# mwhoffman/pybo

Hardware: AMD Instinct MI355X
Metric: BO-step wall-clock (GP fit + 1e6-candidate acq sweep) at N obs; steps/sec (higher is better)
Workload: dtype f64

## Files before the change

pybo_amd/csrc/api.hip:

```cpp
#include <math.h>
#include <stdio.h>
#include <stdlib.h>
#include <string.h>

#include <algorithm>
#include <cmath>
#include <functional>
#include <new>

#include "gpx_internal.h"
#include "gpx_diag.h"
#include "acq_core.h"
#include "mes_math.h"
#include "kg_math.h"

using namespace gpx;

static thread_local std::string g_create_err;

#define HIPCHK(h, call)                                                                     \
    do {                                                                                    \
        hipError_t e_ = (call);                                                             \
        if (e_ != hipSuccess) {                                                             \
            char buf_[512];                                                                 \
// ... 99 lines not shown
    void (*set)(gpx_handle* h, int64_t v);
    bool (*ok)(int64_t v) = nullptr;
    const char* bad_ok = nullptr;
};
template <int gpx_handle::*F>
static void store(gpx_handle* h, int64_t v) { h->*F = (int)v; }
static bool mult128(int64_t v) { return v % 128 == 0; }
static const int64_t BIG = INT64_MAX;
static const char* const TG = "chol_tg*: out of range";
static const char* const TRTRI = "trtri_ahead*: out of range";
static const char* const XBG = "x_bg*: out of range";
static const Option kOptions[] = {
    {"chunk", SHIP, 128, BIG, "chunk must be a positive multiple of 128", [](gpx_handle* h, int64_t v) { h->chunk = v; }, mult128},
    {"super_m", SHIP, 1, 16, "super_m must be 1, 2, 4, 8 or 16", store<&gpx_handle::super_m>, [](int64_t v) { return (v & (v - 1)) == 0; }},
    {"tile_order", SHIP, -1, 31, "tile_order: -1 (by size) or bits 0-1 tile map (0..3), bits 2-4 k-loop schedule (1 .. 7)",
     store<&gpx_handle::tile_order>, [](int64_t v) { return v == -1 || v >= 4; }},
    {"sweep_cache", SHIP, -1, 1, "sweep_cache must be 1, 0 or -1",
     [](gpx_handle* h, int64_t v) { h->cache_on = (v == 1); if (v < 0) { h->cache_valid = false; h->npend = 0; } }},
    {"prune", SHIP, -1, 1, "prune must be -1 (by size and gate), 0 (never) or 1 (wherever legal)", store<&gpx_handle::prune>},
    {"prune_keep", DIAG, 0, 1, "prune_keep must be 0 or 1", store<&gpx_handle::prune_keep>},
    {"prune_bound", DIAG, -1, 2, "prune_bound must be -1 (by guard), 0 (generic kernel), 1 (matrix-pipe kernel) or 2 (fp32 matrix-pipe kernel)", store<&gpx_handle::prune_bound>},
    {"bound_fact", DIAG, 0, 1, "bound_fact must be 0 (the fp32 bound kernel never takes its factorised form) or 1 (by its guard)", store<&gpx_handle::bound_fact>},
    {"prune_rows", DIAG, -1, 1000000, "prune_rows must be -1 (by size), 0 (no second bound) or a number of block rows", store<&gpx_handle::prune_rows>},
    {"short_map", DIAG, -1, 1, "short_map must be -1 (by size), 0 (never) or 1 (wherever tile map 3 is in use)", store<&gpx_handle::short_map>},
    {"chol_w", SHIP, 0, 8, "chol_w must be 0 (by size) or in [2, 8]", store<&gpx_handle::chol_w>, [](int64_t v) { return v != 1; }},
    {"chol_tg", SHIP, -1, 1000000000, TG, store<&gpx_handle::chol_tg>, [](int64_t v) { return v == 0 || v == 1; }, "chol_tg must be 0 or 1"},
    {"chol_tg_chunks", DIAG, -1, 1000000000, TG, store<&gpx_handle::tg_chunks>},
    {"chol_tg_grid", DIAG, -1, 1000000000, TG, store<&gpx_handle::tg_grid>},
    {"chol_tg_trace", DIAG, -1, 1000000000, TG, store<&gpx_handle::tg_trace>},
    {"chol_tg_isolate", DIAG, -1, 1000000000, TG, store<&gpx_handle::tg_isolate>},
    {"chol_tg_nap", DIAG, -1, 1000000000, TG, [](gpx_handle* h, int64_t v) { h->tg_nap = (int)std::max<int64_t>(0, std::min<int64_t>(127, v)); }},
    {"chol_tg_tmo_ms", SHIP, -1, 1000000000, TG, store<&gpx_handle::tg_tmo_ms>},
    {"chol_tg_min", SHIP, -1, 1000000000, TG, [](gpx_handle* h, int64_t v) { h->tg_min = (int)std::max<int64_t>(1, v); }},
    {"chol_tg_max", SHIP, -1, 1000000000, TG, [](gpx_handle* h, int64_t v) { h->tg_max = (int)std::max<int64_t>(1, v); }},
    {"chol_tg_db", SHIP, -1, 1000000000, TG, [](gpx_handle* h, int64_t v) { h->tg_db = (v < 0) ? -1 : (v != 0 ? 1 : 0); }},
    {"chol_tg_db_max", SHIP, -1, 1000000000, TG, [](gpx_handle* h, int64_t v) { h->tg_db_max = (int)std::max<int64_t>(0, v); }},
    {"chol_tg_fuse", SHIP, -1, 1000000000, TG, [](gpx_handle* h, int64_t v) { h->tg_fuse = (v != 0) ? 1 : 0; }},
    {"trtri_ahead", SHIP, 0, 1000000, TRTRI, [](gpx_handle* h, int64_t v) { h->trtri_ahead = (v != 0) ? 1 : 0; }},
    {"trtri_ahead_min", SHIP, 0, 1000000, TRTRI, [](gpx_handle* h, int64_t v) { h->trtri_ahead_min = (int)std::max<int64_t>(4, v); }},
    {"chol_fuse", SHIP, 0, 1, "chol_fuse must be 0 or 1", store<&gpx_handle::chol_fuse>},
    {"chol_graph", SHIP, 0, 1, "chol_graph must be 0 or 1", store<&gpx_handle::chol_graph>},
    {"chol_merge", SHIP, 0, 100000, "chol_merge: 0 (off) or a minimum number of block rows", store<&gpx_handle::chol_merge>},
    {"chol_rl", SHIP, 0, 1, "chol_rl must be 0 or 1", store<&gpx_handle::chol_rl>},
    {"x_skip", DIAG, 0, 7, "x_skip: bits 0..2", store<&gpx_handle::x_skip>},
    {"x_bg", DIAG, 0, 10000000, XBG, store<&gpx_handle::x_bg>},
    {"x_bg_lds", DIAG, 0, 10000000, XBG, store<&gpx_handle::x_bg_lds>},
// ... 839 lines not shown
    const int64_t nx = Xc ? M * h->d : 0;
    int rc;
    if ((rc = ensure(h, h->dXc, h->cap_xc, staged_ws(WsCarver(nullptr), nx, M).bytes / 8))) return rc;
    const StagedWs st = staged_ws(WsCarver(h->dXc), nx, M);
    if (Xc) {
        Span sp(h, T_COPY);
        HIPCHK(h, hipMemcpyAsync(st.X, Xc, (size_t)nx * 8, hipMemcpyHostToDevice, h->stream));
    }
    if (sync_upload) HIPCHK(h, hipStreamSynchronize(h->stream));
    if ((rc = core(st.X, acq_all ? st.acq : nullptr, mu ? st.mu : nullptr, s2 ? st.s2 : nullptr))) return rc;
    {
        Span sp(h, T_COPY);
        if (acq_all) HIPCHK(h, hipMemcpyAsync(acq_all, st.acq, (size_t)M * 8, hipMemcpyDeviceToHost, h->stream));
        if (mu) HIPCHK(h, hipMemcpyAsync(mu, st.mu, (size_t)M * 8, hipMemcpyDeviceToHost, h->stream));
        if (s2) HIPCHK(h, hipMemcpyAsync(s2, st.s2, (size_t)M * 8, hipMemcpyDeviceToHost, h->stream));
    }
    HIPCHK(h, hipStreamSynchronize(h->stream));
    return GPX_OK;
}

static const int64_t PRUNE_MIN_M = 32768, PRUNE_MIN_NP = 1024, PRUNE_MAX_SHARE_DIV = 4;
static const double PRUNE_GATE_S2 = 1.0 / 64.0;
static const int PRUNE_ROWS_MIN_NP = 32, PRUNE_ROWS_DIV = 4;

struct PruneGeom { int64_t G, Gg, cap; };
static PruneGeom prune_geom(int nP, int64_t k, int64_t M) {
    const int64_t gen_tiles = std::max<int64_t>(1, 512 / ((nP + 1) / 2));
    const int64_t G0 = (int64_t)TBH * std::min<int64_t>(32, gen_tiles);
    const int64_t G = std::max<int64_t>(G0, (k + TBH - 1) / TBH * TBH);
    return {G, (int64_t)TBH * gen_tiles, std::max<int64_t>(G, M / PRUNE_MAX_SHARE_DIV)};
}

static int prune_ws(gpx_handle* h, int64_t M, int64_t cap, int64_t Gg, int64_t extra, PruneWs& w, bool rows = false) {
    const int64_t need = prune_ws_layout(WsCarver(nullptr), M, cap, h->d, h->Np, Gg, extra, rows).bytes;
    if (!h->dprune || need > h->cap_prune) h->ens_rec = gpx_handle::EnsPruneRecord();
    if (int rc = ensure(h, h->dprune, h->cap_prune, need)) return rc;
    w = prune_ws_layout(WsCarver(h->dprune), M, cap, h->d, h->Np, Gg, extra, rows);
    return GPX_OK;
}

static const int64_t BOUND_F32_MIN_M = 131072;
static void bound_dots(gpx_handle* h, const double* dXc, int64_t M, const PruneWs& w, bool bound_mfma, double* out) {
    hipStream_t s = h->stream;
    launch_prune_alpha(s, h->dU, h->Np, h->da, h->rho, h->bias, w.alpha2, w.sabs, w.sc);
    if (bound_mfma)
        launch_bound_mfma(s, h->dXs, h->N, h->Np, (int)h->d, w.alpha2, h->rho, dXc, M, h->dinvell, h->prune_bound, M >= BOUND_F32_MIN_M, h->bound_fact != 0,
                          w.bws, w.sc, out);
    launch_sweep_rank1_v(s, h->dXs, h->N, (int)h->d, w.alpha2, h->Np, w.sc + 2, dXc, M, h->dinvell, h->kernel_id, h->rho,
                         nullptr, out, bound_mfma ? w.sc + 9 : nullptr);
}

static int64_t sweep_chunk(const gpx_handle* h, int64_t M) {
    const int64_t chunk_opt = h->chunk > 0 ? h->chunk : (h->Np <= 4096 ? 131072 : 65536);
    return std::min<int64_t>(chunk_opt, (M + TBH - 1) / TBH * TBH);
}

struct SelectList { const double* X; int64_t* idx; int64_t n; };
struct SelectOps {
    std::function<int(const double* X, int64_t mb, int64_t me, double* out, double* mu, double* s2)> exact;
    std::function<int(int64_t Gg, double* value, bool* go)> gate;
    std::function<int(double* ub, int64_t done)> bound;
    std::function<int()> after_seeds;
    std::function<int(SelectList& list)> refine;
};

template <typename Rec>
static int select_topk_pruned(gpx_handle* L, bool legal, bool selection_only, int acq_id, int n, int nP, int64_t Np_min, const double* dXc,
                              int64_t M, int64_t k, int64_t ws_extra, bool ws_rows, PruneWs& w, PruneHint& hint, Rec& rec, double* out,
                              const SelectOps& ops, int64_t* done) {
    const PruneGeom geom = prune_geom(nP, k, M);
    const int64_t G = geom.G, Gg = geom.Gg, cap = geom.cap;
    const Rec fresh = rec;
    auto start_rec = [&]() {
        rec = fresh;
        rec.path = 0, rec.M = M, rec.k = k, rec.G = G, rec.Gg = Gg, rec.cap = cap, rec.gate = NAN;
    };
    start_rec();
    *done = 0;
    legal = legal && selection_only && acq_id == GPX_ACQ_EI && k > 0 && L->prune != 0 && M >= 3 * G;
    bool pruning = legal && (L->prune == 1 || (M >= PRUNE_MIN_M && Np_min >= PRUNE_MIN_NP && M >= Gg + 2 * G));
    if (!pruning) return GPX_OK;
    hipStream_t s = L->stream;
    int rc;
    const int64_t kk = std::min<int64_t>(k, TOPK_PASS);
    if ((rc = ensure(L, L->dblkv, L->cap_blk, topk_blocks(M) * kk))) return rc;
    if ((rc = ensure(L, L->dblki, L->cap_blki, topk_blocks(M) * kk))) return rc;
    if ((rc = ensure(L, L->dtopv, L->cap_top, (int64_t)TOPK_MAX * 2))) return rc;
    L->dtopi = reinterpret_cast<int64_t*>(L->dtopv + TOPK_MAX);
    if ((rc = prune_ws(L, M, cap, Gg, ws_extra, w, ws_rows))) return rc;
    start_rec();
    PruneHint key;
    key.kernel_id = L->kernel_id, key.n = n, key.d = L->d, key.nP = nP, key.Np_min = Np_min, key.M = M, key.k = k;
    const bool automatic = L->prune < 0;
// ... 122 lines not shown
        h->npend = 0;
        if ((rc = ensure(h, h->dcZ, h->cap_cz, M * h->d))) return rc;
        if ((rc = ensure(h, h->dcq, h->cap_cq, 2 * M))) return rc;
        h->dcp = h->dcq + h->cap_cq / 2;
        cq = h->dcq;
        cp = h->dcp;
        if (dXc != h->dcZ)
            HIPCHK(h, hipMemcpyAsync(h->dcZ, dXc, (size_t)M * h->d * 8, hipMemcpyDeviceToDevice, s));
    }

    const int sweep_order = h->tile_order >= 0 ? h->tile_order : (Np / NB < 32 ? 7 : 19);

    auto run_chunks = [&](const double* X, int64_t mb, int64_t me, double* out, double* mu, double* s2) -> int {
        for (int64_t m0 = mb; m0 < me; m0 += chunk) {
            const int64_t valid = std::min(chunk, me - m0);
            const int64_t cols = (valid + TBH - 1) / TBH * TBH;
            {
                Span sp(h, T_XGRAM);
                launch_cross_gram(s, h->dXs, Np, h->N, (int)h->d, X, m0, me, cols, h->dinvell, h->kernel_id,
                                  h->rho, h->dKs, Np);
            }
            {
                Span sp(h, T_TRMM);
                launch_sweep_trmm(s, h->dU, Np, nP, h->dKs, chunk, cols, h->da, h->dQp, h->dPp, chunk, sweep_order, h->super_m, h->dclk, h->short_map);
            }
            h->tacc[T_NLAUNCH] += 1.0;
            h->tacc[T_FLOP] += (double)h->N * (double)h->N * (double)valid;
            {
                Span sp(h, T_ACQ);
                if (kg) {
                    launch_kg_cross(s, kb.B, Np, h->dKs, Np, cols, h->dkgw, chunk);
                    launch_acq_kg(s, h->dQp, h->dPp, chunk, nP, m0, valid, h->rho, h->bias, h->sn2, h->kernel_id, (int)h->d, X, h->dinvell,
                                  kb.As, kb.m, kb.al, h->dkgw, chunk, out, mu, s2, cq, cp);
                } else if (mes) launch_acq_mes(s, h->dQp, h->dPp, chunk, nP, m0, valid, h->rho, h->bias, ys, out, mu, s2, cq, cp);
                else launch_acq(s, h->dQp, h->dPp, chunk, nP, m0, valid, h->rho, h->bias, acq_id, p0, out, mu, s2, cq, cp);
            }
        }
        return GPX_OK;
    };

    gpx_handle::PruneRecord& rec = h->prune_rec;
    PruneWs w;
    KeepWs kw = {};
    SelectOps ops;
    ops.exact = run_chunks;
    ops.gate = [&](int64_t Gg, double* value, bool* go) -> int {
        run_chunks(dXc, 0, Gg, d_acq, nullptr, w.gs2);
// ... 8 lines not shown
    ops.bound = [&](double* ub, int64_t done) -> int {
        const bool bound_mfma = h->prune_bound != 0 && bound_mfma_ks(h->kernel_id, (int)h->d) > 0;
        {
            Span sp(h, T_BOUND);
            bound_dots(h, dXc, M, w, bound_mfma, w.dots);
            if (h->prune_keep) {
                if ((rc = ensure(h, h->dkeep, h->cap_keep, keep_ws(WsCarver(nullptr), M, rec.G).bytes))) return rc;
                kw = keep_ws(WsCarver(h->dkeep), M, rec.G);
                HIPCHK(h, hipMemcpyAsync(kw.dots, w.dots, (size_t)M * 8, hipMemcpyDeviceToDevice, s));
            }
            launch_prune_ub(s, w.dots, ub, M, done, w.sc, h->rho, h->bias, p0);
        }
        rec.bound_kernel = bound_mfma ? -1 : 0, rec.st = w.st, rec.kept = h->prune_keep != 0;
        if (rec.kept) HIPCHK(h, hipMemcpyAsync(kw.ub, ub, (size_t)M * 8, hipMemcpyDeviceToDevice, s));
        return GPX_OK;
    };
    ops.after_seeds = [&]() -> int {
        if (rec.kept) HIPCHK(h, hipMemcpyAsync(kw.seed, w.idx, (size_t)rec.G * 8, hipMemcpyDeviceToDevice, s));
        return GPX_OK;
    };
    ops.refine = [&](SelectList& list) -> int { return second_bound(h, w, chunk, sweep_order, p0, list); };
    int64_t done = 0;
    const bool legal = !h->cache_on && h->rho >= gpx::S2_FLOOR && h->rho < INFINITY;
    if ((rc = select_topk_pruned(h, legal, selection_only, acq_id, 1, nP, Np, dXc, M, k, 0, true, w, h->prune_hint, rec, d_acq, ops, &done)))
        return rc;
    if ((rc = plain_rest(ops, dXc, done, chunk, M, d_acq, d_mu, d_s2))) return rc;
    if (h->cache_on) {
        h->cache_valid = true;
        h->cache_M = M;
    }
    if (k > 0 && (rc = topk_core(h, d_acq, M, k, top_val, top_idx))) return rc;
    HIPCHK(h, hipGetLastError());
    return GPX_OK;
}

extern "C" int gpx_sweep_dev(gpx_handle* h, int acq_id, const double* params, int nparams, const double* dXc,
                             int64_t M, int64_t k, double* top_val, int64_t* top_idx, double* d_acq_all,
                             double* d_mu, double* d_s2) {
    return guarded(h, [&]() -> int {
        if (!h) return GPX_EARG;
        return sweep_core(h, acq_id, params, nparams, dXc, M, k, top_val, top_idx, d_acq_all, d_mu, d_s2);
    });
}

extern "C" int gpx_sweep(gpx_handle* h, int acq_id, const double* params, int nparams, const double* Xc,
                         int64_t M, int64_t k, double* top_val, int64_t* top_idx, double* acq_all, double* mu,
                         double* s2) {
// ... 588 lines not shown
            PruneWs wm = w;
            if (h != L) {
                h->prune_rec = gpx_handle::PruneRecord();
                if ((rc = prune_ws(h, 0, 0, 0, 0, wm))) return member_fail(L, h, m, rc);
            }
            {
                Span sp(h, T_BOUND);
                const bool bound_mfma = h->prune_bound != 0 && bound_mfma_ks(h->kernel_id, (int)h->d) > 0;
                bound_dots(h, dXc, M, wm, bound_mfma, t1);
                launch_prune_ub_fold(h->stream, t1, ub, M, wm.sc, h->rho, h->bias, params[0], m == 0, delta + m,
                                     bound_mfma ? 1 : 0, delta + n + m);
            }
            HIPCHK(L, hipStreamSynchronize(h->stream));
        }
        {
            Span sp(L, T_BOUND);
            launch_prune_ub_mean(s, ub, M, done, (double)n);
        }
        rec.delta = delta;
        return GPX_OK;
    };
    ops.after_seeds = [&]() -> int { HIPCHK(L, hipStreamSynchronize(s)); return GPX_OK; };
    int64_t done = 0;
    if ((rc = select_topk_pruned(L, members_ok, !d_out && !d_mu && !d_s2, acq_id, n, nPmax, Np_min, dXc, M, k, 3 * n, false, w, L->ens_hint, rec,
                                 out, ops, &done)))
        return rc;
    if ((rc = plain_rest(ops, dXc, done, sweep_chunk(L, M), M, out, d_mu, d_s2))) return rc;
    if (k > 0) {
        if ((rc = topk_core(L, out, M, k, top_val, top_idx))) return rc;
    } else {
        HIPCHK(L, hipStreamSynchronize(L->stream));
    }
    HIPCHK(L, hipGetLastError());
    return GPX_OK;
}

static int ensemble_check(gpx_handle* const* members, int n) {
    if (!members || n < 1 || !members[0]) return GPX_EARG;
    for (int m = 1; m < n; ++m)
        if (!members[m]) {
            members[0]->err = "ensemble_sweep: NULL member handle";
            return GPX_EARG;
        }
    return GPX_OK;
}

extern "C" int gpx_ensemble_predict(gpx_handle* const* members, int n_members, const double* Xc, int64_t M,
// ... 254 lines not shown
```

pybo_amd/csrc/gemm_core.h:

```cpp
#pragma once
#include <hip/hip_runtime.h>
#include <stdint.h>
#include <type_traits>

namespace gpx {

typedef double d4 __attribute__((ext_vector_type(4)));
typedef double d2 __attribute__((ext_vector_type(2)));

constexpr int TB = 128;
constexpr int BK = 16;
constexpr int LDT = TB + 16;
constexpr int GEMM_THREADS = 256;
constexpr int GEMM_LDS_F64 = 2 * 2 * BK * LDT;
constexpr int GEMM_LDS_BYTES = GEMM_LDS_F64 * 8;

__device__ __forceinline__ void acc_zero(d4 (&acc)[4][4]) {
#pragma unroll
    for (int i = 0; i < 4; ++i)
#pragma unroll
        for (int j = 0; j < 4; ++j) acc[i][j] = (d4){0.0, 0.0, 0.0, 0.0};
}

struct LaunchClock {
    const unsigned long long c0, r0;
    __device__ __forceinline__ LaunchClock() : c0(__builtin_readcyclecounter()), r0(wall_clock64()) {}
    __device__ __forceinline__ void add(unsigned long long* clk) const {
        if (clk && threadIdx.x == 0) {
            atomicAdd(clk, (unsigned long long)__builtin_readcyclecounter() - c0);
            atomicAdd(clk + 1, (unsigned long long)wall_clock64() - r0);
        }
    }
};

template <bool PRIO, bool ILV = false>
__device__ __forceinline__ void gemm_tile_128_b(d4 (&acc)[4][4], const double* __restrict__ A, int64_t lda,
                                                const double* __restrict__ B, int64_t ldb, int k_lo,
                                                int k_hi, double* smem) {
    const int t = threadIdx.x;
    const int lane = t & 63;
    const int w = t >> 6;
    const int wm = w >> 1, wn = w & 1;
    double* As = smem;
    double* Bs = smem + 2 * BK * LDT;
// ... 289 lines not shown
            if (W2) {
                ra[kk] = __builtin_bit_cast(d2, __builtin_amdgcn_raw_buffer_load_b128(rA, voA, kk * soA, AUX));
                rb[kk] = __builtin_bit_cast(d2, __builtin_amdgcn_raw_buffer_load_b128(rB, voB, kk * soB, AUX));
                __builtin_amdgcn_sched_group_barrier(0x020, 2, 0);
            }
        }
        if (W2) {
            Abase += (int64_t)BK32 * lda * 8;
            Bbase += (int64_t)BK32 * ldb * 8;
        }
        __syncthreads();
    };
    int kt = 0;
    for (; kt + 2 < nk; ++kt) step(kt, std::true_type{}, std::true_type{});
    if (kt + 1 < nk) { step(kt, std::true_type{}, std::false_type{}); ++kt; }
    step(kt, std::false_type{}, std::false_type{});
    if (PRIO) __builtin_amdgcn_s_setprio(PRIO - 1);
}

typedef __attribute__((address_space(3))) void* gemm_lds_ptr;
template <int BKL>
constexpr int gemm_l_lds_f64() { return 2 * BKL * LDT; }

template <int BKL, int PRIO = 1, int NSET = 2, bool ILV = false, bool TRI = false, bool NEGA = false, int AUX = 0, bool REV = false>
__device__ __forceinline__ void gemm_tile_128_l(d4 (&acc)[4][4], const double* __restrict__ A, int64_t lda,
                                                const double* __restrict__ B, int64_t ldb, int k_lo, int k_hi,
                                                double* smem) {
    static_assert(!TRI || ILV, "TRI needs the interleaved row blocks");
    static_assert(!REV || BKL == 32, "REV is the order of the 32-row steps: gemm_rev32 for other step sizes");
    constexpr int G = BKL / 4;
    const int lane = threadIdx.x & 63;
    const int w = __builtin_amdgcn_readfirstlane(threadIdx.x >> 6);
    const int wm = w >> 1, wn = w & 1;
    double* As = smem;
    double* Bs = smem + BKL * LDT;
    const int nk = (k_hi - k_lo) / BKL;
    if (nk <= 0) return;
    const char* Abase = reinterpret_cast<const char*>(A + (int64_t)(REV ? k_hi - BKL : k_lo) * lda);
    const char* Bbase = reinterpret_cast<const char*>(B + (int64_t)(REV ? k_hi - BKL : k_lo) * ldb);
    const int64_t stepA = (REV ? -1 : 1) * (int64_t)BKL * lda * 8, stepB = (REV ? -1 : 1) * (int64_t)BKL * ldb * 8;
    const int voA = (int)(((int64_t)w * lda + 2 * lane) * 8), voB = (int)(((int64_t)w * ldb + 2 * lane) * 8);
    const int soA = (int)(4 * lda * 8), soB = (int)(4 * ldb * 8);
    auto issue = [&]() {
        __amdgpu_buffer_rsrc_t rA = __builtin_amdgcn_make_buffer_rsrc((void*)Abase, 0, -1, 0x00020000);
        __amdgpu_buffer_rsrc_t rB = __builtin_amdgcn_make_buffer_rsrc((void*)Bbase, 0, -1, 0x00020000);
#pragma unroll
        for (int p = 0; p < BKL / 4; ++p) {
            __builtin_amdgcn_raw_ptr_buffer_load_lds(rA, (gemm_lds_ptr)(As + (w + 4 * p) * LDT), 16, voA, p * soA, 0, AUX);
            __builtin_amdgcn_raw_ptr_buffer_load_lds(rB, (gemm_lds_ptr)(Bs + (w + 4 * p) * LDT), 16, voB, p * soB, 0, AUX);
        }
        Abase += stepA;
        Bbase += stepB;
    };
    const int fr = lane & 15, fk = lane >> 4;
    constexpr int IST = ILV ? 32 : 16;
    const double* as = As + (ILV ? wm * 16 : wm * 64) + fr + fk * LDT;
    const double* bs = Bs + wn * 64 + fr + fk * LDT;
    auto step = [&](auto i0c, bool more) {
        constexpr int I0 = decltype(i0c)::value;
        asm volatile("s_waitcnt vmcnt(0)" ::: "memory");
        __builtin_amdgcn_s_barrier();
        asm volatile("" ::: "memory");
        if (PRIO) __builtin_amdgcn_s_setprio(PRIO);
        double a[NSET][4], b[NSET][4];
        auto frag = [&](int set, int g) {
#pragma unroll
            for (int i = I0; i < 4; ++i) a[set][i] = as[g * 4 * LDT + i * IST];
#pragma unroll
            for (int j = 0; j < 4; ++j) b[set][j] = bs[g * 4 * LDT + j * 16];
        };
        frag(0, 0);
#pragma unroll
        for (int kk = 0; kk < G; ++kk) {
            if (PRIO && kk == G / 2) __builtin_amdgcn_s_setprio(PRIO + 1);
            if (NSET == 2 && kk + 1 < G) {
                frag((kk + 1) & 1, kk + 1);
                __builtin_amdgcn_sched_group_barrier(0x100, 8 - I0, 0);
            }
#pragma unroll
            for (int i = I0; i < 4; ++i)
#pragma unroll
                for (int j = 0; j < 4; ++j)
                    acc[i][j] = __builtin_amdgcn_mfma_f64_16x16x4f64(a[kk % NSET][i], b[kk % NSET][j], acc[i][j], 0, 0, NEGA ? 1 : 0);
            __builtin_amdgcn_sched_group_barrier(0x008, 4 * (4 - I0), 0);
            if (NSET == 1 && kk + 1 < G) frag(0, kk + 1);
        }
        if (PRIO) __builtin_amdgcn_s_setprio(0);
        asm volatile("s_waitcnt lgkmcnt(0)" ::: "memory");
        __builtin_amdgcn_s_barrier();
        if (more) issue();
    };
    issue();
    if (!TRI) {
        for (int kt = 0; kt < nk; ++kt) step(std::integral_constant<int, 0>{}, kt + 1 < nk);
    } else {
        constexpr int Q = 32 / BKL;
        const int nd = nk - 3 * Q;
        if (!REV) {
            for (int kt = 0; kt < nd; ++kt) step(std::integral_constant<int, 0>{}, true);
            for (int q = 0; q < Q; ++q) step(std::integral_constant<int, 1>{}, true);
            for (int q = 0; q < Q; ++q) step(std::integral_constant<int, 2>{}, true);
            for (int q = 0; q < Q; ++q) step(std::integral_constant<int, 3>{}, q + 1 < Q);
        } else {
            for (int q = 0; q < Q; ++q) step(std::integral_constant<int, 3>{}, true);
            for (int q = 0; q < Q; ++q) step(std::integral_constant<int, 2>{}, true);
            for (int q = 0; q < Q; ++q) step(std::integral_constant<int, 1>{}, true);
            for (int kt = 0; kt < nd; ++kt) step(std::integral_constant<int, 0>{}, kt + 1 < nd);
// ... 299 lines not shown
```

pybo_amd/csrc/gpx_internal.h:

```cpp
#pragma once
#include <hip/hip_runtime.h>
#include <stdint.h>
#include <string>
#include <vector>

#include "../../include/gpx.h"
#include "prune_hint.h"
#include "ws_layout.h"

namespace gpx {

constexpr int DMAX_RFF = DMAX;
constexpr int DMAX_RFF_RESIDENT = 64;
constexpr int TOPK_MAX = 4096;
constexpr int TOPK_PASS = 64;

enum Timer {
    T_GRAM = 0, T_CHOL, T_TRTRI, T_ALPHA, T_XGRAM, T_TRMM, T_ACQ, T_RFF, T_NLAUNCH, T_FLOP, T_COPY, T_APPEND,
    T_RANK1, T_RFFSWEEP, T_RFFOPS, T_TGFALL, T_SCLK, T_RFFCLK, T_AHEAD, T_BOUND, T_BATCH, T_JOINT, T_COUNT
};

struct EventPair { hipEvent_t a, b; int slot; };

struct EnsBatchMember {
// ... 134 lines not shown
    };
    struct PruneRecord : SelectRecord {
        const int* st = nullptr;
        int bound_kernel = -1;
        bool kept = false;
        int nR = 0;
        int64_t nsurv2 = 0;
        const double *qR = nullptr, *ub2 = nullptr;
        const int64_t* idx2 = nullptr;
    } prune_rec;
    struct EnsPruneRecord : SelectRecord {
        int n = 0;
        const double* delta = nullptr;
    } ens_rec;
    gpx::PruneHint prune_hint, ens_hint;
    int prune_keep = 0;
    int prune_bound = -1;
#ifdef GPX_BOUND32_NOFACT
    int bound_fact = 0;
#else
    int bound_fact = 1;
#endif
    int prune_rows = -1;
    int short_map = -1;
    char* dkeep = nullptr;
    int64_t cap_keep = 0;

    const double* app_w = nullptr;
    bool cache_on = false;
    bool cache_valid = false;
    int64_t cache_M = 0;
    double* dcZ = nullptr;
    double* dcq = nullptr;
    double* dcp = nullptr;
    int64_t cap_cz = 0, cap_cq = 0;
    double* dpend = nullptr;
    int64_t pend_ld = 0;
    int npend = 0;

    bool spec_active = false;
    bool spec_launched = false;
    bool spec_used = false;
    bool apply_pending = false;
    uint64_t gen = 0, spec_gen = 0;
    std::vector<double> spec_x;
    double* dspec = nullptr;
// ... 39 lines not shown
int ensure_side_streams(gpx_handle* h);
void launch_cholesky(gpx_handle* h);
bool launch_cholesky_tg(gpx_handle* h);
int tg_abort_code(gpx_handle* h);
int64_t tg_trace_copy(gpx_handle* h, long long* out, int64_t n);
void tg_free(gpx_handle* h);
int64_t tg_tasks_copy(int nP, int chunks, int16_t* out, int64_t cap, int64_t* counts);
void launch_trtri(gpx_handle* h);
void launch_trtri_ahead(gpx_handle* h, hipStream_t s, int top);
int trtri_top(int nP);
void launch_refine_inverse(gpx_handle* h, double* tmp);
void launch_alpha(gpx_handle* h);
void launch_kinv_diag(gpx_handle* h, double* out);
void launch_transpose_lower(hipStream_t s, const double* R, int64_t Np, double* out, int64_t N);
void launch_cholesky_small(hipStream_t s, double* S, double* R, int64_t np, int* flag);
void launch_posterior_wide(hipStream_t s, const double* A, const double* v, const double* z, int n, int64_t np, double sc,
                           double sn2, double* B, double* R, double* work, int* flag, double* theta);

void launch_cross_gram(hipStream_t s, const double* Xs, int64_t rows, int64_t N, int d, const double* Xc,
                       int64_t m0, int64_t M, int64_t cols, const double* invell, int kernel_id,
                       double rho, double* Ks, int64_t ldk);
void launch_sweep_trmm(hipStream_t s, const double* U, int64_t Np, int nR, const double* Ks, int64_t ldk,
                       int64_t cols, const double* a, double* Qp, double* Pp, int64_t ldp,
                       int tile_order, int super_m, unsigned long long* clk, int short_map = -1);
void launch_acq(hipStream_t s, const double* Qp, const double* Pp, int64_t ldp, int nrb, int64_t m0,
                int64_t cols_valid, double rho, double bias, int acq_id, double p0, double* acq_out,
                double* mu_out, double* s2_out, double* qsum, double* psum);
struct MesArg;
void launch_acq_mes(hipStream_t s, const double* Qp, const double* Pp, int64_t ldp, int nrb, int64_t m0,
                    int64_t cols_valid, double rho, double bias, const MesArg& ys, double* acq_out,
                    double* mu_out, double* s2_out, double* qsum, double* psum);
void launch_kg_solve(hipStream_t s, const double* U, int64_t Np, int64_t N, int m, const double* V, double* W);
void launch_kg_cross(hipStream_t s, const double* B, int64_t Np, const double* Ks, int64_t ldk, int64_t cols, double* C, int64_t ldc);
void launch_acq_kg(hipStream_t s, const double* Qp, const double* Pp, int64_t ldp, int nrb, int64_t m0, int64_t cols_valid,
                   double rho, double bias, double sn2, int kid, int d, const double* X, const double* invell, const double* As, int m,
                   const double* al, const double* C, int64_t ldc, double* acq_out, double* mu_out, double* s2_out, double* qsum,
                   double* psum);
void launch_kg_point_sums(hipStream_t s, const double* Xs, int64_t N, int d, const double* Z, int np, const double* invell, int kid,
                          double rho, const double* B, const double* alpha, const double* Wz, const double* Vz, double* S);
void launch_kg_point_final(hipStream_t s, const double* S, int np, int d, const double* Z, const double* invell, const double* As,
                           int m, const double* al, int kid, double rho, double bias, double sn2, double* L, double* f, double* g);
void launch_pend_store(hipStream_t s, const double* w, int64_t Nj, int64_t ldw, const double* scal, double* row,
                       double* pscal_j);
void launch_cache_apply(hipStream_t s, const double* v, const double* scal, int64_t M, double* qsum, double* psum);
void launch_scale_point(hipStream_t s, const double* x, const double* invell, int d, double* xs);
void launch_sweep_rank1_v(hipStream_t s, const double* Xs, int64_t Ntot, int d, const double* Wq, int64_t ldw,
                          const double* pscal, const double* Z, int64_t M, const double* invell, int kernel_id,
// ... 100 lines not shown
```

pybo_amd/csrc/kernels_sweep.hip:

```cpp
#include "acq_core_dev.h"
#include "gemm_core.h"
#include "gpx_internal.h"
#include "gpx_math.h"
#include "bound_exp.h"
#include "bound_f32.h"
#include "sweep_map.h"

namespace gpx {

constexpr int XK = 64, XN = 128, XDC = 16;

template <bool FIRST>
__device__ __forceinline__ void dist_step(const double (*xo)[XK], const double (*xc)[XN], int k, int ty, int tx,
                                          double (&r2)[8][4]) {
    double a8[8], b4[4];
#pragma unroll
    for (int a = 0; a < 8; ++a) a8[a] = xo[k][ty * 8 + a];
#pragma unroll
    for (int b = 0; b < 4; ++b) b4[b] = xc[k][tx * 4 + b];
#pragma unroll
    for (int a = 0; a < 8; ++a)
#pragma unroll
        for (int b = 0; b < 4; ++b) {
            const double df = a8[a] - b4[b];
// ... 64 lines not shown
}

void launch_cross_gram(hipStream_t s, const double* Xs, int64_t rows, int64_t N, int d, const double* Xc,
                       int64_t m0, int64_t M, int64_t cols, const double* invell, int kernel_id,
                       double rho, double* Ks, int64_t ldk) {
    const int64_t Np = rows;
    const int64_t tiles = Np / XK;
    const int XRTa = (kernel_id == GPX_KERN_SE_ARD && d <= XDC) ? 1 : XRT;
    const int XRTv = XRTa;
    dim3 grid((unsigned)((tiles + XRTa - 1) / XRTa), (unsigned)(cols / XN));
#define GPX_CG(KID) \
    hipLaunchKernelGGL(k_cross_gram<KID>, grid, dim3(256), 0, s, Xs, N, Np, d, Xc, m0, M, invell, rho, Ks, ldk, XRTv)
    switch (kernel_id) {
        case GPX_KERN_SE_ARD: GPX_CG(GPX_KERN_SE_ARD); break;
        case GPX_KERN_MATERN52: GPX_CG(GPX_KERN_MATERN52); break;
        case GPX_KERN_MATERN32: GPX_CG(GPX_KERN_MATERN32); break;
        default: GPX_CG(GPX_KERN_MATERN12); break;
    }
#undef GPX_CG
}

__device__ __forceinline__ bool sweep_tile_rev(int mt, int nP) { return nP >= 32 && 2 * mt < nP - 1; }

template <bool ILV = false>
__device__ __forceinline__ void sweep_epilogue(const d4 (&acc)[4][4], const double* __restrict__ avec, int64_t m0,
                                               double* __restrict__ Qrow, double* __restrict__ Prow, double* red) {
    const int lane = threadIdx.x & 63, w = threadIdx.x >> 6;
    const int wm = w >> 1, wn = w & 1;
    double qs[4] = {0.0, 0.0, 0.0, 0.0}, ps[4] = {0.0, 0.0, 0.0, 0.0};
#pragma unroll
    for (int i = 0; i < 4; ++i) {
        double av[4];
#pragma unroll
        for (int r = 0; r < 4; ++r) av[r] = avec[m0 + (ILV ? (2 * i + wm) * 16 : wm * 64 + i * 16) + (lane >> 4) + 4 * r];
#pragma unroll
        for (int j = 0; j < 4; ++j)
#pragma unroll
            for (int r = 0; r < 4; ++r) {
                const double v = acc[i][j][r];
                qs[j] = fma(v, v, qs[j]);
                ps[j] = fma(v, av[r], ps[j]);
            }
    }
#pragma unroll
    for (int j = 0; j < 4; ++j) {
        double q = qs[j], p = ps[j];
        q += __shfl_xor(q, 16);
        p += __shfl_xor(p, 16);
        q += __shfl_xor(q, 32);
        p += __shfl_xor(p, 32);
        qs[j] = q;
        ps[j] = p;
    }
    if (lane < 16) {
#pragma unroll
        for (int j = 0; j < 4; ++j) {
            const int c = wn * 64 + j * 16 + lane;
            red[(wm * TB + c) * 2 + 0] = qs[j];
            red[(wm * TB + c) * 2 + 1] = ps[j];
        }
    }
    __syncthreads();
    if (threadIdx.x < TB) {
        const int c = threadIdx.x;
        Qrow[c] = red[c * 2] + red[(TB + c) * 2];
        Prow[c] = red[c * 2 + 1] + red[(TB + c) * 2 + 1];
    }
}

template <int RES, class Loop>
__device__ __forceinline__ void sweep_tiles(int b, const double* __restrict__ U, int64_t Np, const double* __restrict__ Ks, int NT,
                                            int nR, const double* __restrict__ avec, double* __restrict__ Qp, double* __restrict__ Pp,
                                            int64_t ldp, int order, int sm, unsigned long long* clk, double* smem, Loop loop) {
    const LaunchClock lc;
    const int nP = (int)(Np / TB);
    int mt, nt, mt2;
    if (!sweep_tile_of<RES>(b, order, sm, NT, nR, mt, nt, mt2)) return;
#pragma unroll 1
    for (int ph = 0; ph < 2; ++ph) {
        if (ph == 1) {
            if (mt2 < 0) break;
            mt = mt2;
            __syncthreads();
        }
        const int64_t m0 = (int64_t)mt * TB, n0 = (int64_t)nt * TB;
        d4 acc[4][4];
        acc_zero(acc);
        loop(acc, U + m0, Ks + (int64_t)nt * Np * TB, (mt + 1) * TB, sweep_tile_rev(mt, nP));
        sweep_epilogue<true>(acc, avec, m0, Qp + (int64_t)mt * ldp + n0, Pp + (int64_t)mt * ldp + n0, smem);
    }
    lc.add(clk);
}

template <int VAR>
__global__ __launch_bounds__(GEMM_THREADS, 2) void k_sweep_trmm(const double* __restrict__ U, int64_t Np,
                                                                const double* __restrict__ Ks,
                                                                int64_t ldk, int NT, int nR,
                                                                const double* __restrict__ avec,
                                                                double* __restrict__ Qp,
                                                                double* __restrict__ Pp, int64_t ldp,
                                                                int order, int sm, unsigned long long* clk) {
    __shared__ __attribute__((aligned(16))) double smem[GEMM_LDS_F64];
    sweep_tiles<64>(blockIdx.x, U, Np, Ks, NT, nR, avec, Qp, Pp, ldp, order, sm, clk, smem,
                    [&](d4 (&acc)[4][4], const double* At, const double* Bt, int kend, bool rev) {
        if (!rev) {
            if (VAR == 2) gemm_tile_128_b<true, true>(acc, At, Np, Bt, TB, 0, kend, smem);
            else if (VAR == 5) gemm_tile_128_g<1, false, true>(acc, At, Np, Bt, TB, 0, kend, smem);
            else gemm_tile_128_s<1, false, true>(acc, At, Np, Bt, TB, 0, kend, smem);
        } else {
            if (VAR == 2) gemm_rev32(0, kend, [&](int k0, int k1) { gemm_tile_128_b<true, true>(acc, At, Np, Bt, TB, k0, k1, smem); });
            else if (VAR == 5) gemm_tile_128_g<1, false, true, true>(acc, At, Np, Bt, TB, 0, kend, smem);
            else gemm_tile_128_s<1, false, true, true>(acc, At, Np, Bt, TB, 0, kend, smem);
        }
    });
}

template <int BKL, int WGS, int PRIO, int NSET, bool TRI, int AUX = 0, bool DOWN = true>
__global__ __launch_bounds__(GEMM_THREADS, WGS) void k_sweep_trmm_l(const double* __restrict__ U, int64_t Np,
                                                                    const double* __restrict__ Ks, int64_t ldk, int NT, int nR,
                                                                    const double* __restrict__ avec,
                                                                    double* __restrict__ Qp, double* __restrict__ Pp,
                                                                    int64_t ldp, int order, int sm,
                                                                    unsigned long long* clk, int b0) {
    __shared__ __attribute__((aligned(16))) double smem[gemm_l_lds_f64<BKL>()];
    sweep_tiles<32 * WGS>((int)blockIdx.x + b0, U, Np, Ks, NT, nR, avec, Qp, Pp, ldp, order, sm, clk, smem,
                          [&](d4 (&acc)[4][4], const double* At, const double* Bt, int kend, bool rev) {
        if (!(DOWN && rev)) gemm_tile_128_l<BKL, PRIO, NSET, true, TRI, false, AUX>(acc, At, Np, Bt, TB, 0, kend, smem);
        else if constexpr (BKL == 32) gemm_tile_128_l<32, PRIO, NSET, true, TRI, false, AUX, true>(acc, At, Np, Bt, TB, 0, kend, smem);
        else gemm_rev32(0, kend, [&](int k0, int k1) { gemm_tile_128_l<BKL, PRIO, NSET, true, false, false, AUX>(acc, At, Np, Bt, TB, k0, k1, smem); });
    });
}

__global__ __launch_bounds__(GEMM_THREADS, 2) void k_sweep_trmm_w(const double* __restrict__ U, int64_t Np,
                                                                  const double* __restrict__ Ks, int64_t ldk, int NT, int nR,
                                                                  const double* __restrict__ avec, double* __restrict__ Qp,
                                                                  double* __restrict__ Pp, int64_t ldp, int order, int sm,
                                                                  unsigned long long* clk) {
    __shared__ __attribute__((aligned(16))) double smem[4 * GEMM_W_IMG_F64];
    sweep_tiles<64>(blockIdx.x, U, Np, Ks, NT, nR, avec, Qp, Pp, ldp, order, sm, clk, smem,
                    [&](d4 (&acc)[4][4], const double* At, const double* Bt, int kend, bool rev) {
        if (!rev) gemm_tile_128_w<1, 1, false, true, 0, true>(acc, At, Np, Bt, TB, 0, kend, smem);
        else gemm_rev32(0, kend, [&](int k0, int k1) { gemm_tile_128_w<1, 1, false, true, 0, false>(acc, At, Np, Bt, TB, k0, k1, smem); });
    });
}

template <int RES>
static int sweep_order_of(int order, int short_map, int sm, int NT) {
    if (order != 3 || short_map == 0) return order;
    if (short_map < 0 && !sweep_map_is_short<RES>(sm, NT)) return order;
    return short_map == 2 ? SWEEP_ORDER_SHORT_STRIDED : SWEEP_ORDER_SHORT;
}

void launch_sweep_trmm(hipStream_t s, const double* U, int64_t Np, int nR, const double* Ks, int64_t ldk,
                       int64_t cols, const double* a, double* Qp, double* Pp, int64_t ldp,
                       int tile_order, int super_m, unsigned long long* clk, int short_map) {
    const int NT = (int)(cols / TB);
    const int order0 = tile_order & 3, var = (tile_order >> 2) & 7;
#define GPX_SW(K) hipLaunchKernelGGL(K, dim3(nblk), dim3(GEMM_THREADS), 0, s, U, Np, Ks, ldk, NT, nR, a, Qp, Pp, ldp, order, super_m, clk)
#define GPX_SWL(K) hipLaunchKernelGGL(K, dim3(nblk), dim3(GEMM_THREADS), 0, s, U, Np, Ks, ldk, NT, nR, a, Qp, Pp, ldp, order, super_m, clk, 0)
    if (var == 7) {
        const int order = sweep_order_of<96>(order0, short_map, super_m, NT);
        const unsigned nblk = sweep_grid<96>(order, super_m, NT, nR);
        GPX_SWL((k_sweep_trmm_l<16, 3, 1, 2, false>));
    } else if (var == 1) {
        const int order = sweep_order_of<64>(order0, short_map, super_m, NT);
        const unsigned nblk = sweep_grid<64>(order, super_m, NT, nR);
        GPX_SW(k_sweep_trmm_w);
    } else if (var == 4 || var == 3) {
        const int order = sweep_order_of<64>(order0, short_map, super_m, NT);
        const unsigned nblk = sweep_grid<64>(order, super_m, NT, nR);
#ifdef GPX_SWEEP_PROBES
        const int aux = tile_order >> 5;
        if (var == 4 && aux == 1) GPX_SWL((k_sweep_trmm_l<32, 2, 1, 2, true, 1>));
        else if (var == 4 && aux == 2) GPX_SWL((k_sweep_trmm_l<32, 2, 1, 2, true, 2>));
        else if (var == 4 && aux == 3) GPX_SWL((k_sweep_trmm_l<32, 2, 1, 2, true, 16>));
        else if (var == 4 && aux == 4) GPX_SWL((k_sweep_trmm_l<32, 2, 1, 2, true, 17>));
        else if (var == 4 && aux == 5) GPX_SWL((k_sweep_trmm_l<32, 2, 1, 2, true, 3>));
        else if (var == 4 && aux == 6) GPX_SWL((k_sweep_trmm_l<32, 2, 1, 2, true, 0, false>));
        else if (var == 4 && aux == 7) {
            for (unsigned g0 = 0; g0 < nblk; g0 += 512)
                hipLaunchKernelGGL((k_sweep_trmm_l<32, 2, 1, 2, true>), dim3(nblk - g0 < 512 ? nblk - g0 : 512), dim3(GEMM_THREADS), 0, s, U, Np, Ks, ldk, NT, nR, a,
                                   Qp, Pp, ldp, order, super_m, clk, (int)g0);
        }
        else
#endif
        if (var == 4) GPX_SWL((k_sweep_trmm_l<32, 2, 1, 2, true>));
        else GPX_SWL((k_sweep_trmm_l<32, 2, 1, 2, false>));
    } else {
        const int order = sweep_order_of<64>(order0, short_map, super_m, NT);
        const unsigned nblk = sweep_grid<64>(order, super_m, NT, nR);
// ... 938 lines not shown
```

Before: 83.09.

## Add narrow-column sweep tiles and smaller prune seed batches for large Np

```diff
diff --git a/pybo_amd/csrc/api.hip b/pybo_amd/csrc/api.hip
--- a/pybo_amd/csrc/api.hip
+++ b/pybo_amd/csrc/api.hip
@@ -145,6 +145,9 @@
     {"prune_bound", DIAG, -1, 2, "prune_bound must be -1 (by guard), 0 (generic kernel), 1 (matrix-pipe kernel) or 2 (fp32 matrix-pipe kernel)", store<&gpx_handle::prune_bound>},
     {"bound_fact", DIAG, 0, 1, "bound_fact must be 0 (the fp32 bound kernel never takes its factorised form) or 1 (by its guard)", store<&gpx_handle::bound_fact>},
     {"prune_rows", DIAG, -1, 1000000, "prune_rows must be -1 (by size), 0 (no second bound) or a number of block rows", store<&gpx_handle::prune_rows>},
+    {"sweep_cols", SHIP, -1, 128, "sweep_cols must be -1 (by size), 128, 64 or 32", store<&gpx_handle::sweep_cols>,
+     [](int64_t v) { return v == -1 || v == 128 || v == 64 || v == 32; }},
+    {"prune_seeds", DIAG, 0, 1000000, "prune_seeds must be 0 (by the rule) or a number of seeds", store<&gpx_handle::prune_seeds>},
     {"short_map", DIAG, -1, 1, "short_map must be -1 (by size), 0 (never) or 1 (wherever tile map 3 is in use)", store<&gpx_handle::short_map>},
     {"chol_w", SHIP, 0, 8, "chol_w must be 0 (by size) or in [2, 8]", store<&gpx_handle::chol_w>, [](int64_t v) { return v != 1; }},
     {"chol_tg", SHIP, -1, 1000000000, TG, store<&gpx_handle::chol_tg>, [](int64_t v) { return v == 0 || v == 1; }, "chol_tg must be 0 or 1"},
@@ -1030,11 +1033,17 @@
 static const int64_t PRUNE_MIN_M = 32768, PRUNE_MIN_NP = 1024, PRUNE_MAX_SHARE_DIV = 4;
 static const double PRUNE_GATE_S2 = 1.0 / 64.0;
 static const int PRUNE_ROWS_MIN_NP = 32, PRUNE_ROWS_DIV = 4;
+static const int PRUNE_SEEDS_MIN_NP = SWEEP_NARROW_MIN_NP;
+static bool seeds_narrow(const gpx_handle* h) {
+    return h->Np / NB >= PRUNE_SEEDS_MIN_NP && (h->tile_order < 0 || h->tile_order == 19) && h->sweep_cols != 128;
+}
 
 struct PruneGeom { int64_t G, Gg, cap; };
-static PruneGeom prune_geom(int nP, int64_t k, int64_t M) {
+static PruneGeom prune_geom(int nP, int64_t k, int64_t M, bool narrow = false, int64_t seeds = 0) {
     const int64_t gen_tiles = std::max<int64_t>(1, 512 / ((nP + 1) / 2));
-    const int64_t G0 = (int64_t)TBH * std::min<int64_t>(32, gen_tiles);
+    int64_t G0 = (int64_t)TBH * std::min<int64_t>(32, gen_tiles);
+    if (narrow && M >= PRUNE_MIN_M) G0 = 32 * std::max<int64_t>(1, 256 / ((nP + 1) / 2));
+    if (seeds > 0) G0 = (seeds + 31) / 32 * 32;
     const int64_t G = std::max<int64_t>(G0, (k + TBH - 1) / TBH * TBH);
     return {G, (int64_t)TBH * gen_tiles, std::max<int64_t>(G, M / PRUNE_MAX_SHARE_DIV)};
 }
@@ -1073,10 +1082,10 @@
 };
 
 template <typename Rec>
-static int select_topk_pruned(gpx_handle* L, bool legal, bool selection_only, int acq_id, int n, int nP, int64_t Np_min, const double* dXc,
-                              int64_t M, int64_t k, int64_t ws_extra, bool ws_rows, PruneWs& w, PruneHint& hint, Rec& rec, double* out,
-                              const SelectOps& ops, int64_t* done) {
-    const PruneGeom geom = prune_geom(nP, k, M);
+static int select_topk_pruned(gpx_handle* L, bool legal, bool selection_only, int acq_id, int n, int nP, int64_t Np_min, bool narrow,
+                              const double* dXc, int64_t M, int64_t k, int64_t ws_extra, bool ws_rows, PruneWs& w, PruneHint& hint, Rec& rec,
+                              double* out, const SelectOps& ops, int64_t* done) {
+    const PruneGeom geom = prune_geom(nP, k, M, narrow, L->prune_seeds);
     const int64_t G = geom.G, Gg = geom.Gg, cap = geom.cap;
     const Rec fresh = rec;
     auto start_rec = [&]() {
@@ -1245,7 +1254,8 @@
             }
             {
                 Span sp(h, T_TRMM);
-                launch_sweep_trmm(s, h->dU, Np, nP, h->dKs, chunk, cols, h->da, h->dQp, h->dPp, chunk, sweep_order, h->super_m, h->dclk, h->short_map);
+                launch_sweep_trmm(s, h->dU, Np, nP, h->dKs, chunk, cols, h->da, h->dQp, h->dPp, chunk, sweep_order, h->super_m, h->dclk, h->short_map,
+                                  valid, h->sweep_cols);
             }
             h->tacc[T_NLAUNCH] += 1.0;
             h->tacc[T_FLOP] += (double)h->N * (double)h->N * (double)valid;
@@ -1300,7 +1310,7 @@
     ops.refine = [&](SelectList& list) -> int { return second_bound(h, w, chunk, sweep_order, p0, list); };
     int64_t done = 0;
     const bool legal = !h->cache_on && h->rho >= gpx::S2_FLOOR && h->rho < INFINITY;
-    if ((rc = select_topk_pruned(h, legal, selection_only, acq_id, 1, nP, Np, dXc, M, k, 0, true, w, h->prune_hint, rec, d_acq, ops, &done)))
+    if ((rc = select_topk_pruned(h, legal, selection_only, acq_id, 1, nP, Np, seeds_narrow(h), dXc, M, k, 0, true, w, h->prune_hint, rec, d_acq, ops, &done)))
         return rc;
     if ((rc = plain_rest(ops, dXc, done, chunk, M, d_acq, d_mu, d_s2))) return rc;
     if (h->cache_on) {
@@ -1935,7 +1945,7 @@
     };
     ops.after_seeds = [&]() -> int { HIPCHK(L, hipStreamSynchronize(s)); return GPX_OK; };
     int64_t done = 0;
-    if ((rc = select_topk_pruned(L, members_ok, !d_out && !d_mu && !d_s2, acq_id, n, nPmax, Np_min, dXc, M, k, 3 * n, false, w, L->ens_hint, rec,
+    if ((rc = select_topk_pruned(L, members_ok, !d_out && !d_mu && !d_s2, acq_id, n, nPmax, Np_min, false, dXc, M, k, 3 * n, false, w, L->ens_hint, rec,
                                  out, ops, &done)))
         return rc;
     if ((rc = plain_rest(ops, dXc, done, sweep_chunk(L, M), M, out, d_mu, d_s2))) return rc;
diff --git a/pybo_amd/csrc/gemm_core.h b/pybo_amd/csrc/gemm_core.h
--- a/pybo_amd/csrc/gemm_core.h
+++ b/pybo_amd/csrc/gemm_core.h
@@ -15,11 +15,12 @@
 constexpr int GEMM_LDS_F64 = 2 * 2 * BK * LDT;
 constexpr int GEMM_LDS_BYTES = GEMM_LDS_F64 * 8;
 
-__device__ __forceinline__ void acc_zero(d4 (&acc)[4][4]) {
+template <int NJ>
+__device__ __forceinline__ void acc_zero(d4 (&acc)[4][NJ]) {
 #pragma unroll
     for (int i = 0; i < 4; ++i)
 #pragma unroll
-        for (int j = 0; j < 4; ++j) acc[i][j] = (d4){0.0, 0.0, 0.0, 0.0};
+        for (int j = 0; j < NJ; ++j) acc[i][j] = (d4){0.0, 0.0, 0.0, 0.0};
 }
 
 struct LaunchClock {
@@ -355,10 +356,11 @@
 template <int BKL>
 constexpr int gemm_l_lds_f64() { return 2 * BKL * LDT; }
 
-template <int BKL, int PRIO = 1, int NSET = 2, bool ILV = false, bool TRI = false, bool NEGA = false, int AUX = 0, bool REV = false>
-__device__ __forceinline__ void gemm_tile_128_l(d4 (&acc)[4][4], const double* __restrict__ A, int64_t lda,
+template <int BKL, int PRIO = 1, int NSET = 2, bool ILV = false, bool TRI = false, bool NEGA = false, int AUX = 0, bool REV = false, int NJ = 4>
+__device__ __forceinline__ void gemm_tile_128_l(d4 (&acc)[4][NJ], const double* __restrict__ A, int64_t lda,
                                                 const double* __restrict__ B, int64_t ldb, int k_lo, int k_hi,
-                                                double* smem) {
+                                                double* smem, int bcol = 0) {
+    static_assert(NJ == 4 || NJ == 2 || NJ == 1, "a wave owns 4, 2 or 1 column groups");
     static_assert(!TRI || ILV, "TRI needs the interleaved row blocks");
     static_assert(!REV || BKL == 32, "REV is the order of the 32-row steps: gemm_rev32 for other step sizes");
     constexpr int G = BKL / 4;
@@ -388,19 +390,19 @@
     const int fr = lane & 15, fk = lane >> 4;
     constexpr int IST = ILV ? 32 : 16;
     const double* as = As + (ILV ? wm * 16 : wm * 64) + fr + fk * LDT;
-    const double* bs = Bs + wn * 64 + fr + fk * LDT;
+    const double* bs = Bs + bcol + wn * (16 * NJ) + fr + fk * LDT;
     auto step = [&](auto i0c, bool more) {
         constexpr int I0 = decltype(i0c)::value;
         asm volatile("s_waitcnt vmcnt(0)" ::: "memory");
         __builtin_amdgcn_s_barrier();
         asm volatile("" ::: "memory");
         if (PRIO) __builtin_amdgcn_s_setprio(PRIO);
-        double a[NSET][4], b[NSET][4];
+        double a[NSET][4], b[NSET][NJ];
         auto frag = [&](int set, int g) {
 #pragma unroll
             for (int i = I0; i < 4; ++i) a[set][i] = as[g * 4 * LDT + i * IST];
 #pragma unroll
-            for (int j = 0; j < 4; ++j) b[set][j] = bs[g * 4 * LDT + j * 16];
+            for (int j = 0; j < NJ; ++j) b[set][j] = bs[g * 4 * LDT + j * 16];
         };
         frag(0, 0);
 #pragma unroll
@@ -408,14 +410,14 @@
             if (PRIO && kk == G / 2) __builtin_amdgcn_s_setprio(PRIO + 1);
             if (NSET == 2 && kk + 1 < G) {
                 frag((kk + 1) & 1, kk + 1);
-                __builtin_amdgcn_sched_group_barrier(0x100, 8 - I0, 0);
+                __builtin_amdgcn_sched_group_barrier(0x100, 4 + NJ - I0, 0);
             }
 #pragma unroll
             for (int i = I0; i < 4; ++i)
 #pragma unroll
-                for (int j = 0; j < 4; ++j)
+                for (int j = 0; j < NJ; ++j)
                     acc[i][j] = __builtin_amdgcn_mfma_f64_16x16x4f64(a[kk % NSET][i], b[kk % NSET][j], acc[i][j], 0, 0, NEGA ? 1 : 0);
-            __builtin_amdgcn_sched_group_barrier(0x008, 4 * (4 - I0), 0);
+            __builtin_amdgcn_sched_group_barrier(0x008, NJ * (4 - I0), 0);
             if (NSET == 1 && kk + 1 < G) frag(0, kk + 1);
         }
         if (PRIO) __builtin_amdgcn_s_setprio(0);
diff --git a/pybo_amd/csrc/gpx_internal.h b/pybo_amd/csrc/gpx_internal.h
--- a/pybo_amd/csrc/gpx_internal.h
+++ b/pybo_amd/csrc/gpx_internal.h
@@ -180,6 +180,8 @@
     int bound_fact = 1;
 #endif
     int prune_rows = -1;
+    int sweep_cols = -1;
+    int prune_seeds = 0;
     int short_map = -1;
     char* dkeep = nullptr;
     int64_t cap_keep = 0;
@@ -265,7 +267,9 @@
                        double rho, double* Ks, int64_t ldk);
 void launch_sweep_trmm(hipStream_t s, const double* U, int64_t Np, int nR, const double* Ks, int64_t ldk,
                        int64_t cols, const double* a, double* Qp, double* Pp, int64_t ldp,
-                       int tile_order, int super_m, unsigned long long* clk, int short_map = -1);
+                       int tile_order, int super_m, unsigned long long* clk, int short_map = -1, int64_t valid = -1, int sweep_cols = 128);
+int sweep_cols_of(int sweep_cols, int tile_order, int nP, int nR, int64_t valid);
+constexpr int SWEEP_NARROW_MIN_NP = 48;
 void launch_acq(hipStream_t s, const double* Qp, const double* Pp, int64_t ldp, int nrb, int64_t m0,
                 int64_t cols_valid, double rho, double bias, int acq_id, double p0, double* acq_out,
                 double* mu_out, double* s2_out, double* qsum, double* psum);
diff --git a/pybo_amd/csrc/kernels_sweep.hip b/pybo_amd/csrc/kernels_sweep.hip
--- a/pybo_amd/csrc/kernels_sweep.hip
+++ b/pybo_amd/csrc/kernels_sweep.hip
@@ -110,19 +110,19 @@
 
 __device__ __forceinline__ bool sweep_tile_rev(int mt, int nP) { return nP >= 32 && 2 * mt < nP - 1; }
 
-template <bool ILV = false>
-__device__ __forceinline__ void sweep_epilogue(const d4 (&acc)[4][4], const double* __restrict__ avec, int64_t m0,
+template <bool ILV = false, int NJ = 4>
+__device__ __forceinline__ void sweep_epilogue(const d4 (&acc)[4][NJ], const double* __restrict__ avec, int64_t m0,
                                                double* __restrict__ Qrow, double* __restrict__ Prow, double* red) {
     const int lane = threadIdx.x & 63, w = threadIdx.x >> 6;
     const int wm = w >> 1, wn = w & 1;
-    double qs[4] = {0.0, 0.0, 0.0, 0.0}, ps[4] = {0.0, 0.0, 0.0, 0.0};
+    double qs[NJ] = {}, ps[NJ] = {};
 #pragma unroll
     for (int i = 0; i < 4; ++i) {
         double av[4];
 #pragma unroll
         for (int r = 0; r < 4; ++r) av[r] = avec[m0 + (ILV ? (2 * i + wm) * 16 : wm * 64 + i * 16) + (lane >> 4) + 4 * r];
 #pragma unroll
-        for (int j = 0; j < 4; ++j)
+        for (int j = 0; j < NJ; ++j)
 #pragma unroll
             for (int r = 0; r < 4; ++r) {
                 const double v = acc[i][j][r];
@@ -131,7 +131,7 @@
             }
     }
 #pragma unroll
-    for (int j = 0; j < 4; ++j) {
+    for (int j = 0; j < NJ; ++j) {
         double q = qs[j], p = ps[j];
         q += __shfl_xor(q, 16);
         p += __shfl_xor(p, 16);
@@ -142,21 +142,21 @@
     }
     if (lane < 16) {
 #pragma unroll
-        for (int j = 0; j < 4; ++j) {
-            const int c = wn * 64 + j * 16 + lane;
+        for (int j = 0; j < NJ; ++j) {
+            const int c = wn * (16 * NJ) + j * 16 + lane;
             red[(wm * TB + c) * 2 + 0] = qs[j];
             red[(wm * TB + c) * 2 + 1] = ps[j];
         }
     }
     __syncthreads();
-    if (threadIdx.x < TB) {
+    if (threadIdx.x < 32 * NJ) {
         const int c = threadIdx.x;
         Qrow[c] = red[c * 2] + red[(TB + c) * 2];
         Prow[c] = red[c * 2 + 1] + red[(TB + c) * 2 + 1];
     }
 }
 
-template <int RES, class Loop>
+template <int RES, int NJ = 4, class Loop>
 __device__ __forceinline__ void sweep_tiles(int b, const double* __restrict__ U, int64_t Np, const double* __restrict__ Ks, int NT,
                                             int nR, const double* __restrict__ avec, double* __restrict__ Qp, double* __restrict__ Pp,
                                             int64_t ldp, int order, int sm, unsigned long long* clk, double* smem, Loop loop) {
@@ -171,11 +171,11 @@
             mt = mt2;
             __syncthreads();
         }
-        const int64_t m0 = (int64_t)mt * TB, n0 = (int64_t)nt * TB;
-        d4 acc[4][4];
+        const int64_t m0 = (int64_t)mt * TB, n0 = (int64_t)nt * (32 * NJ);
+        d4 acc[4][NJ];
         acc_zero(acc);
-        loop(acc, U + m0, Ks + (int64_t)nt * Np * TB, (mt + 1) * TB, sweep_tile_rev(mt, nP));
-        sweep_epilogue<true>(acc, avec, m0, Qp + (int64_t)mt * ldp + n0, Pp + (int64_t)mt * ldp + n0, smem);
+        loop(acc, U + m0, Ks + (n0 / TB) * Np * TB, (mt + 1) * TB, sweep_tile_rev(mt, nP), (int)(n0 % TB));
+        sweep_epilogue<true, NJ>(acc, avec, m0, Qp + (int64_t)mt * ldp + n0, Pp + (int64_t)mt * ldp + n0, smem);
     }
     lc.add(clk);
 }
@@ -190,7 +190,7 @@
                                                                 int order, int sm, unsigned long long* clk) {
     __shared__ __attribute__((aligned(16))) double smem[GEMM_LDS_F64];
     sweep_tiles<64>(blockIdx.x, U, Np, Ks, NT, nR, avec, Qp, Pp, ldp, order, sm, clk, smem,
-                    [&](d4 (&acc)[4][4], const double* At, const double* Bt, int kend, bool rev) {
+                    [&](d4 (&acc)[4][4], const double* At, const double* Bt, int kend, bool rev, int) {
         if (!rev) {
             if (VAR == 2) gemm_tile_128_b<true, true>(acc, At, Np, Bt, TB, 0, kend, smem);
             else if (VAR == 5) gemm_tile_128_g<1, false, true>(acc, At, Np, Bt, TB, 0, kend, smem);
@@ -203,7 +203,7 @@
     });
 }
 
-template <int BKL, int WGS, int PRIO, int NSET, bool TRI, int AUX = 0, bool DOWN = true>
+template <int BKL, int WGS, int PRIO, int NSET, bool TRI, int AUX = 0, bool DOWN = true, int NJ = 4>
 __global__ __launch_bounds__(GEMM_THREADS, WGS) void k_sweep_trmm_l(const double* __restrict__ U, int64_t Np,
                                                                     const double* __restrict__ Ks, int64_t ldk, int NT, int nR,
                                                                     const double* __restrict__ avec,
@@ -211,10 +211,11 @@
                                                                     int64_t ldp, int order, int sm,
                                                                     unsigned long long* clk, int b0) {
     __shared__ __attribute__((aligned(16))) double smem[gemm_l_lds_f64<BKL>()];
-    sweep_tiles<32 * WGS>((int)blockIdx.x + b0, U, Np, Ks, NT, nR, avec, Qp, Pp, ldp, order, sm, clk, smem,
-                          [&](d4 (&acc)[4][4], const double* At, const double* Bt, int kend, bool rev) {
-        if (!(DOWN && rev)) gemm_tile_128_l<BKL, PRIO, NSET, true, TRI, false, AUX>(acc, At, Np, Bt, TB, 0, kend, smem);
-        else if constexpr (BKL == 32) gemm_tile_128_l<32, PRIO, NSET, true, TRI, false, AUX, true>(acc, At, Np, Bt, TB, 0, kend, smem);
+    static_assert(NJ == 4 || BKL == 32, "narrow tiles: the 32-row k-step only");
+    sweep_tiles<32 * WGS, NJ>((int)blockIdx.x + b0, U, Np, Ks, NT, nR, avec, Qp, Pp, ldp, order, sm, clk, smem,
+                              [&](d4 (&acc)[4][NJ], const double* At, const double* Bt, int kend, bool rev, int bcol) {
+        if (!(DOWN && rev)) gemm_tile_128_l<BKL, PRIO, NSET, true, TRI, false, AUX>(acc, At, Np, Bt, TB, 0, kend, smem, bcol);
+        else if constexpr (BKL == 32) gemm_tile_128_l<32, PRIO, NSET, true, TRI, false, AUX, true>(acc, At, Np, Bt, TB, 0, kend, smem, bcol);
         else gemm_rev32(0, kend, [&](int k0, int k1) { gemm_tile_128_l<BKL, PRIO, NSET, true, false, false, AUX>(acc, At, Np, Bt, TB, k0, k1, smem); });
     });
 }
@@ -226,7 +227,7 @@
                                                                   unsigned long long* clk) {
     __shared__ __attribute__((aligned(16))) double smem[4 * GEMM_W_IMG_F64];
     sweep_tiles<64>(blockIdx.x, U, Np, Ks, NT, nR, avec, Qp, Pp, ldp, order, sm, clk, smem,
-                    [&](d4 (&acc)[4][4], const double* At, const double* Bt, int kend, bool rev) {
+                    [&](d4 (&acc)[4][4], const double* At, const double* Bt, int kend, bool rev, int) {
         if (!rev) gemm_tile_128_w<1, 1, false, true, 0, true>(acc, At, Np, Bt, TB, 0, kend, smem);
         else gemm_rev32(0, kend, [&](int k0, int k1) { gemm_tile_128_w<1, 1, false, true, 0, false>(acc, At, Np, Bt, TB, k0, k1, smem); });
     });
@@ -239,10 +240,19 @@
     return short_map == 2 ? SWEEP_ORDER_SHORT_STRIDED : SWEEP_ORDER_SHORT;
 }
 
+static const int64_t SWEEP_COLS32_MAX = 512, SWEEP_COLS64_MAX = 1024;
+int sweep_cols_of(int sweep_cols, int tile_order, int nP, int nR, int64_t valid) {
+    if (tile_order < 0 || ((tile_order >> 2) & 7) != 4 || (tile_order >> 5) != 0) return TB;
+    if (sweep_cols > 0) return sweep_cols;
+    if (nP < SWEEP_NARROW_MIN_NP || nR != nP || (tile_order & 3) != 3) return TB;
+    return valid <= SWEEP_COLS32_MAX ? 32 : valid <= SWEEP_COLS64_MAX ? 64 : TB;
+}
+
 void launch_sweep_trmm(hipStream_t s, const double* U, int64_t Np, int nR, const double* Ks, int64_t ldk,
                        int64_t cols, const double* a, double* Qp, double* Pp, int64_t ldp,
-                       int tile_order, int super_m, unsigned long long* clk, int short_map) {
+                       int tile_order, int super_m, unsigned long long* clk, int short_map, int64_t valid, int sweep_cols) {
     const int NT = (int)(cols / TB);
+    if (valid < 0 || valid > cols) valid = cols;
     const int order0 = tile_order & 3, var = (tile_order >> 2) & 7;
 #define GPX_SW(K) hipLaunchKernelGGL(K, dim3(nblk), dim3(GEMM_THREADS), 0, s, U, Np, Ks, ldk, NT, nR, a, Qp, Pp, ldp, order, super_m, clk)
 #define GPX_SWL(K) hipLaunchKernelGGL(K, dim3(nblk), dim3(GEMM_THREADS), 0, s, U, Np, Ks, ldk, NT, nR, a, Qp, Pp, ldp, order, super_m, clk, 0)
@@ -254,6 +264,14 @@
         const int order = sweep_order_of<64>(order0, short_map, super_m, NT);
         const unsigned nblk = sweep_grid<64>(order, super_m, NT, nR);
         GPX_SW(k_sweep_trmm_w);
+    } else if (const int W = sweep_cols_of(sweep_cols, tile_order, (int)(Np / TB), nR, valid); W < TB) {
+        const int NTn = (int)((valid + W - 1) / W);
+        const int order = sweep_order_of<64>(order0, short_map, super_m, NTn);
+        const unsigned nblk = sweep_grid<64>(order, super_m, NTn, nR);
+#define GPX_SWN(K) hipLaunchKernelGGL(K, dim3(nblk), dim3(GEMM_THREADS), 0, s, U, Np, Ks, ldk, NTn, nR, a, Qp, Pp, ldp, order, super_m, clk, 0)
+        if (W == 64) GPX_SWN((k_sweep_trmm_l<32, 2, 1, 2, true, 0, true, 2>));
+        else GPX_SWN((k_sweep_trmm_l<32, 2, 1, 2, true, 0, true, 1>));
+#undef GPX_SWN
     } else if (var == 4 || var == 3) {
         const int order = sweep_order_of<64>(order0, short_map, super_m, NT);
         const unsigned nblk = sweep_grid<64>(order, super_m, NT, nR);
```

New measurement: 86.86, median of 6. +4.5%, better.
